# tanishqkumar/ssd

Measured on NVIDIA H100. Metric: decode tokens/sec (sync speculative decoding, accept-len reported), higher is better.
Workload: dtype bf16

## Files before the change

### ssd_b200/csrc/draft_stream.cuh

```cuda
#pragma once
#include "common.cuh"
#include "sampling.cuh"

namespace ssdk {

constexpr int kDsConsumers = 256;
constexpr int kDsWarps = kDsConsumers / 32;
constexpr int kDsThreads = kDsConsumers + 32;
constexpr int kDsMaxLayers = 32;
constexpr int kDsSplits = 16;
constexpr int kDsShortSplits = 8;
constexpr int kDsLongCtx = 256;
constexpr int kDsSlotBytes = 32768;
constexpr int kDsMaxSlots = 6;
constexpr int kDsMaxSteps = 8;
constexpr int kDsBtSmem = 32;

struct DsLayer {
  const __nv_bfloat16 *qkv, *o, *gate_up, *down, *in_norm, *post_norm, *q_norm, *k_norm;
};

struct DsParams {
  int d, L, H, KV, ffn, vocab, qk_norm;
  float eps, scale_log2;
// ... 11 lines not shown
  float* attn_part;
  __nv_bfloat16* logits;
  long long logits_ld;
  const float* temp;
  const uint64_t* dyn;
  uint64_t seed, call_base;
  ArgMax* samp_partial;
  unsigned* bar_state;
  unsigned* attn_ticket;
  int n_slots;
  DsLayer layers[kDsMaxLayers];
  const int64_t* pend_tok;
  __nv_bfloat16* vec_row0;
  const float* fp8_scale[kDsMaxLayers][4];
};

struct DsVecs {
  __nv_bfloat16 *qkv, *attn, *o, *down, *resid0, *resid1, *act;
  SSDK_DEVINL __nv_bfloat16* resid(int i) const { return i ? resid1 : resid0; }
};
SSDK_DEVINL DsVecs ds_row0_vecs(const DsParams& p, int hd) {
  DsVecs v{};
  __nv_bfloat16* b = p.vec_row0;
  if (!b) return v;
  v.qkv = b; b += ((p.H + 2 * p.KV) * hd + 7) / 8 * 8;
  v.attn = b; b += p.H * hd;
  v.o = b; b += p.d;
  v.down = b; b += p.d;
  v.resid0 = b; b += p.d;
  v.resid1 = b; b += p.d;
  v.act = b;
  return v;
}
__host__ SSDK_DEVINL int ds_xs_floats(int d, int ffn, int q_width) {
  const int a = 2 * d > ffn ? 2 * d : ffn;
  return a > q_width ? a : q_width;
}

SSDK_DEVINL void ds_sync() {
#ifdef SSDK_HOST_EMU
  ::emu::named_barrier(1, kDsConsumers);
#else
  asm volatile("bar.sync 1, 256;" ::: "memory");
#endif
}

struct DsGridBar {
  unsigned long long* counter;
  unsigned long long target;
  __device__ void init() {
    if (threadIdx.x == 0) {
      const unsigned long long c = ld_relaxed_gpu_u64(counter);
      target = c - c % (unsigned long long)gridDim.x;
    }
  }
  __device__ void sync() {
    ds_sync();
    if (threadIdx.x == 0) {
      target += (unsigned long long)gridDim.x;
      red_add_release_gpu_u64(counter, 1ull);
      const long long t0 = clock64();
      while (ld_relaxed_gpu_u64(counter) < target) {
        if (clock64() - t0 > 4000000000LL) __trap();
      }
      fence_acq_rel_gpu();
    }
    ds_sync();
  }
};
// ... 86 lines not shown
    const int parts = g.kind == DS_PAIR ? 2 : 1;
    for (int q = 0; q < parts; ++q) {
      const unsigned slot = n % S, round = n / S;
      mbar_wait(&empty[slot], (round & 1u) ^ 1u);
      mbar_arrive_expect_tx(&full[slot], bytes);
      const void* src = w + ((size_t)(q ? g.rows : 0) + (size_t)c.s * g.rpj) * g.K;
      if constexpr (FP8) {
        if (c.m != DS_HEAD)
          src = reinterpret_cast<const uint8_t*>(w) + ((size_t)(q ? g.rows : 0) + (size_t)c.s * g.rpj) * g.K;
      }
      bulk_load_g2s(ring + (size_t)slot * kDsSlotBytes, src, bytes, &full[slot]);
      ++n;
    }
    ds_cursor_next(p, geom, c);
  }
}

struct DsRing {
  uint8_t* base;
  uint64_t *full, *empty;
  unsigned n_slots;
  unsigned taken;
};
SSDK_DEVINL const uint8_t* ds_acquire(DsRing& r, unsigned k) {
  const unsigned n = r.taken + k, slot = n % r.n_slots;
  mbar_wait(&r.full[slot], (n / r.n_slots) & 1u);
  return r.base + (size_t)slot * kDsSlotBytes;
}
SSDK_DEVINL void ds_release(DsRing& r, unsigned k, int lane) {
  __syncwarp();
  if (lane == 0) mbar_arrive(&r.empty[(r.taken + k) % r.n_slots]);
}

SSDK_DEVINL void ds_load_x(const float* xseg, int steps, int lane, float (&xr)[kDsMaxSteps][8]) {
#pragma unroll
  for (int j = 0; j < kDsMaxSteps; ++j) {
    if (j < steps) {
      const float4 a = *reinterpret_cast<const float4*>(xseg + j * 256 + lane * 8);
      const float4 b = *reinterpret_cast<const float4*>(xseg + j * 256 + lane * 8 + 4);
      xr[j][0] = a.x; xr[j][1] = a.y; xr[j][2] = a.z; xr[j][3] = a.w;
      xr[j][4] = b.x; xr[j][5] = b.y; xr[j][6] = b.z; xr[j][7] = b.w;
    } else {
#pragma unroll
      for (int e = 0; e < 8; ++e) xr[j][e] = 0.f;
    }
  }
}
SSDK_DEVINL float ds_dot_seg(const uint8_t* wseg, int steps, int lane, const float (&xr)[kDsMaxSteps][8]) {
  const uint4* wp = reinterpret_cast<const uint4*>(wseg) + lane;
  float a0 = 0.f, a1 = 0.f, a2 = 0.f, a3 = 0.f;
#pragma unroll
  for (int j = 0; j < kDsMaxSteps; ++j) {
    if (j < steps) {
      const uint4 w = wp[j * 32];
      float2 f = ds_bf2(w.x);
      a0 = fmaf(f.x, xr[j][0], a0); a1 = fmaf(f.y, xr[j][1], a1);
      f = ds_bf2(w.y);
      a2 = fmaf(f.x, xr[j][2], a2); a3 = fmaf(f.y, xr[j][3], a3);
      f = ds_bf2(w.z);
      a0 = fmaf(f.x, xr[j][4], a0); a1 = fmaf(f.y, xr[j][5], a1);
      f = ds_bf2(w.w);
      a2 = fmaf(f.x, xr[j][6], a2); a3 = fmaf(f.y, xr[j][7], a3);
    }
  }
  return warp_sum((a0 + a1) + (a2 + a3));
}

SSDK_DEVINL float2 ds_e4m3x2(uint32_t v) {
#ifdef SSDK_HOST_EMU
  auto one = [](uint32_t b) {
    const int e = (int)((b >> 3) & 15u), m = (int)(b & 7u);
    float x = (e == 15 && m == 7) ? NAN : (e ? std::ldexp(1.0f + (float)m / 8.0f, e - 7) : std::ldexp((float)m, -9));
    return (b & 0x80u) ? -x : x;
  };
// ... 9 lines not shown
  const uint2* wp = reinterpret_cast<const uint2*>(wseg) + lane;
  float a0 = 0.f, a1 = 0.f, a2 = 0.f, a3 = 0.f;
#pragma unroll
  for (int j = 0; j < kDsMaxSteps; ++j) {
    if (j < steps) {
      const uint2 w = wp[j * 32];
      float2 f = ds_e4m3x2(w.x);
      a0 = fmaf(f.x, xr[j][0], a0); a1 = fmaf(f.y, xr[j][1], a1);
      f = ds_e4m3x2(w.x >> 16);
      a2 = fmaf(f.x, xr[j][2], a2); a3 = fmaf(f.y, xr[j][3], a3);
      f = ds_e4m3x2(w.y);
      a0 = fmaf(f.x, xr[j][4], a0); a1 = fmaf(f.y, xr[j][5], a1);
      f = ds_e4m3x2(w.y >> 16);
      a2 = fmaf(f.x, xr[j][6], a2); a3 = fmaf(f.y, xr[j][7], a3);
    }
  }
  return warp_sum((a0 + a1) + (a2 + a3));
}

struct DsSample {
  bool greedy;
  float invT;
  uint64_t seed, call_id;
  ArgMax best;
};
SSDK_DEVINL float ds_score(const DsSample& s, float logit, int idx) {
  if (s.greedy) return logit;
  const uint4 rnd = philox_draw((uint32_t)(idx >> 2), 0u, s.call_id, TAG_SAMPLE, s.seed);
  const float e = u32_to_exp1(u4_word(rnd, idx & 3)) + 1e-10f;
  return logit * s.invT - __logf(e);
}

struct DsRow0 {
  const float* xs;
  const __nv_bfloat16* xg;
  __nv_bfloat16* y;
};
SSDK_DEVINL float ds_dot_seg0(const uint8_t* wseg, int steps, int lane, const float* x0) {
  const uint4* wp = reinterpret_cast<const uint4*>(wseg) + lane;
  float a0 = 0.f, a1 = 0.f, a2 = 0.f, a3 = 0.f;
#pragma unroll 2
  for (int j = 0; j < steps; ++j) {
    const float4 u = *reinterpret_cast<const float4*>(x0 + j * 256 + lane * 8);
    const float4 v = *reinterpret_cast<const float4*>(x0 + j * 256 + lane * 8 + 4);
    const uint4 w = wp[j * 32];
    float2 f = ds_bf2(w.x);
    a0 = fmaf(f.x, u.x, a0); a1 = fmaf(f.y, u.y, a1);
    f = ds_bf2(w.y);
    a2 = fmaf(f.x, u.z, a2); a3 = fmaf(f.y, u.w, a3);
    f = ds_bf2(w.z);
    a0 = fmaf(f.x, v.x, a0); a1 = fmaf(f.y, v.y, a1);
    f = ds_bf2(w.w);
    a2 = fmaf(f.x, v.z, a2); a3 = fmaf(f.y, v.w, a3);
  }
  return warp_sum((a0 + a1) + (a2 + a3));
}
SSDK_DEVINL float ds_dot_seg08(const uint8_t* wseg, int steps, int lane, const float* x0) {
  const uint2* wp = reinterpret_cast<const uint2*>(wseg) + lane;
  float a0 = 0.f, a1 = 0.f, a2 = 0.f, a3 = 0.f;
#pragma unroll 2
  for (int j = 0; j < steps; ++j) {
    const float4 u = *reinterpret_cast<const float4*>(x0 + j * 256 + lane * 8);
    const float4 v = *reinterpret_cast<const float4*>(x0 + j * 256 + lane * 8 + 4);
    const uint2 w = wp[j * 32];
    float2 f = ds_e4m3x2(w.x);
    a0 = fmaf(f.x, u.x, a0); a1 = fmaf(f.y, u.y, a1);
    f = ds_e4m3x2(w.x >> 16);
    a2 = fmaf(f.x, u.z, a2); a3 = fmaf(f.y, u.w, a3);
    f = ds_e4m3x2(w.y);
    a0 = fmaf(f.x, v.x, a0); a1 = fmaf(f.y, v.y, a1);
    f = ds_e4m3x2(w.y >> 16);
    a2 = fmaf(f.x, v.z, a2); a3 = fmaf(f.y, v.w, a3);
  }
  return warp_sum((a0 + a1) + (a2 + a3));
}
SSDK_DEVINL void ds_load_vec(const __nv_bfloat16* v, int n, float* xs);
SSDK_DEVINL const float* ds_row0_x(const DsRow0& r, float* xs, int n) {
  if (r.xs) return r.xs;
  ds_sync();
  ds_load_vec(r.xg, n, xs);
  return xs;
}

template <bool HEAD, bool TWO = false>
SSDK_DEVINL void ds_consume_plain(DsRing& ring, const DsGeom& g, float* xs, __nv_bfloat16* y, DsSample* smp,
                                  const DsRow0& r0 = DsRow0{}) {
  static_assert(!(HEAD && TWO), "row 0 has no lm_head");
  if ((int)blockIdx.x >= g.nj) return;
  const int warp = threadIdx.x >> 5, lane = threadIdx.x & 31;
  const int steps = g.K >> 8;
  float xr[kDsMaxSteps][8];
  ds_load_x(xs, steps, lane, xr);
  const float* x0 = nullptr;
  if constexpr (TWO) x0 = ds_row0_x(r0, xs, g.K);
  for (int s = (int)blockIdx.x; s < g.nj; s += (int)gridDim.x) {
    const uint8_t* st = ds_acquire(ring, 0);
    const float acc = ds_dot_seg(st + (size_t)warp * g.K * 2, steps, lane, xr);
    float acc0 = 0.f;
    if constexpr (TWO) acc0 = ds_dot_seg0(st + (size_t)warp * g.K * 2, steps, lane, x0);
    ds_release(ring, 0, lane);
    ring.taken += 1u;
    const int row = s * 8 + warp;
    if (lane == 0 && row < g.rows) {
      const __nv_bfloat16 o = f2bf(acc);
      if (!HEAD) {
        y[row] = o;
        if constexpr (TWO) r0.y[row] = f2bf(acc0);
      } else {
        if (y) y[row] = o;
        smp->best = argmax_better(smp->best, ArgMax{ds_score(*smp, bf2f(o), row), row});
      }
    }
  }
}
SSDK_DEVINL float ds_silu_mul(float gate, float up) {
  gate = bf16_round(gate);
  up = bf16_round(up);
  return (gate / (1.0f + __expf(-gate))) * up;
}
template <bool TWO>
SSDK_DEVINL void ds_consume_pair(DsRing& ring, const DsGeom& g, float* xs, __nv_bfloat16* act, const DsRow0& r0) {
  if ((int)blockIdx.x >= g.nj) return;
  const int warp = threadIdx.x >> 5, lane = threadIdx.x & 31;
  const int steps = g.K >> 8;
  float xr[kDsMaxSteps][8];
  ds_load_x(xs, steps, lane, xr);
  const float* x0 = nullptr;
  if constexpr (TWO) x0 = ds_row0_x(r0, xs, g.K);
  for (int s = (int)blockIdx.x; s < g.nj; s += (int)gridDim.x) {
    float gate0 = 0.f, up0 = 0.f;
    const uint8_t* sg = ds_acquire(ring, 0);
    const float gate = ds_dot_seg(sg + (size_t)warp * g.K * 2, steps, lane, xr);
    if constexpr (TWO) gate0 = ds_dot_seg0(sg + (size_t)warp * g.K * 2, steps, lane, x0);
    ds_release(ring, 0, lane);
    const uint8_t* su = ds_acquire(ring, 1);
    const float up = ds_dot_seg(su + (size_t)warp * g.K * 2, steps, lane, xr);
    if constexpr (TWO) up0 = ds_dot_seg0(su + (size_t)warp * g.K * 2, steps, lane, x0);
    ds_release(ring, 1, lane);
    ring.taken += 2u;
    const int i = s * 8 + warp;
    if (lane == 0 && i < g.rows) {
      act[i] = f2bf(ds_silu_mul(gate, up));
      if constexpr (TWO) r0.y[i] = f2bf(ds_silu_mul(gate0, up0));
    }
  }
}
template <bool TWO>
SSDK_DEVINL void ds_consume_split(DsRing& ring, const DsGeom& g, float* xs, float* res, __nv_bfloat16* y,
                                  const DsRow0& r0) {
  if ((int)blockIdx.x >= g.nj) return;
  const int warp = threadIdx.x >> 5, lane = threadIdx.x & 31;
  const int row_in_job = warp / g.segs, seg = warp - row_in_job * g.segs;
  const int seg_len = g.K / g.segs, steps = seg_len >> 8;
  float xr[kDsMaxSteps][8];
  ds_load_x(xs + seg * seg_len, steps, lane, xr);
  const float* x0 = nullptr;
  if constexpr (TWO) x0 = ds_row0_x(r0, xs, g.K);
  const size_t w_off = ((size_t)row_in_job * g.K + (size_t)seg * seg_len) * 2;
  unsigned it = 0;
  for (int s = (int)blockIdx.x; s < g.nj; s += (int)gridDim.x, ++it) {
    const uint8_t* st = ds_acquire(ring, 0);
    const float acc = ds_dot_seg(st + w_off, steps, lane, xr);
    float acc0 = 0.f;
    if constexpr (TWO) acc0 = ds_dot_seg0(st + w_off, steps, lane, x0 + seg * seg_len);
    ds_release(ring, 0, lane);
    ring.taken += 1u;
    float* rb = res + (it & 1u) * kDsWarps;
    float* rb0 = rb + 2 * kDsWarps;
    if (lane == 0) {
      rb[warp] = acc;
      if constexpr (TWO) rb0[warp] = acc0;
    }
    ds_sync();
    if ((int)threadIdx.x < g.rpj) {
      const int row = s * g.rpj + (int)threadIdx.x;
      if (row < g.rows) {
        float v = 0.f;
        for (int q = 0; q < g.segs; ++q) v += rb[(int)threadIdx.x * g.segs + q];
        y[row] = f2bf(v);
        if constexpr (TWO) {
          float v0 = 0.f;
          for (int q = 0; q < g.segs; ++q) v0 += rb0[(int)threadIdx.x * g.segs + q];
          r0.y[row] = f2bf(v0);
        }
      }
    }
  }
}

template <bool TWO>
SSDK_DEVINL void ds_consume_plain8(DsRing& ring, const DsGeom& g, float* xs, __nv_bfloat16* y, const DsRow0& r0,
                                   const float* scale) {
  if ((int)blockIdx.x >= g.nj) return;
  const int warp = threadIdx.x >> 5, lane = threadIdx.x & 31;
  const int steps = g.K >> 8;
  float xr[kDsMaxSteps][8];
  ds_load_x(xs, steps, lane, xr);
  const float* x0 = nullptr;
  if constexpr (TWO) x0 = ds_row0_x(r0, xs, g.K);
  for (int s = (int)blockIdx.x; s < g.nj; s += (int)gridDim.x) {
    const int ra = s * 16 + warp, rb = ra + 8;
    const float sa = ra < g.rows ? scale[ra] : 0.f, sb = rb < g.rows ? scale[rb] : 0.f;
    const uint8_t* wa = ds_acquire(ring, 0) + (size_t)warp * g.K;
    const uint8_t* wb = wa + (size_t)8 * g.K;
    const float acc_a = ds_dot_seg8(wa, steps, lane, xr);
    const float acc_b = ds_dot_seg8(wb, steps, lane, xr);
    float acc0_a = 0.f, acc0_b = 0.f;
    if constexpr (TWO) {
      acc0_a = ds_dot_seg08(wa, steps, lane, x0);
      acc0_b = ds_dot_seg08(wb, steps, lane, x0);
    }
    ds_release(ring, 0, lane);
    ring.taken += 1u;
    if (lane == 0) {
      if (ra < g.rows) {
        y[ra] = f2bf(acc_a * sa);
        if constexpr (TWO) r0.y[ra] = f2bf(acc0_a * sa);
      }
      if (rb < g.rows) {
        y[rb] = f2bf(acc_b * sb);
        if constexpr (TWO) r0.y[rb] = f2bf(acc0_b * sb);
      }
    }
  }
}
template <bool TWO>
SSDK_DEVINL void ds_consume_pair8(DsRing& ring, const DsGeom& g, float* xs, __nv_bfloat16* act, const DsRow0& r0,
                                  const float* scale) {
  if ((int)blockIdx.x >= g.nj) return;
  const int warp = threadIdx.x >> 5, lane = threadIdx.x & 31;
  const int steps = g.K >> 8;
  float xr[kDsMaxSteps][8];
  ds_load_x(xs, steps, lane, xr);
  const float* x0 = nullptr;
  if constexpr (TWO) x0 = ds_row0_x(r0, xs, g.K);
  for (int s = (int)blockIdx.x; s < g.nj; s += (int)gridDim.x) {
    const int ia = s * 16 + warp, ib = ia + 8;
    const float sga = ia < g.rows ? scale[ia] : 0.f, sua = ia < g.rows ? scale[g.rows + ia] : 0.f;
    const float sgb = ib < g.rows ? scale[ib] : 0.f, sub = ib < g.rows ? scale[g.rows + ib] : 0.f;
    float ga0 = 0.f, gb0 = 0.f, ua0 = 0.f, ub0 = 0.f;
    const uint8_t* sg = ds_acquire(ring, 0) + (size_t)warp * g.K;
    const float ga = ds_dot_seg8(sg, steps, lane, xr);
    const float gb = ds_dot_seg8(sg + (size_t)8 * g.K, steps, lane, xr);
    if constexpr (TWO) {
      ga0 = ds_dot_seg08(sg, steps, lane, x0);
      gb0 = ds_dot_seg08(sg + (size_t)8 * g.K, steps, lane, x0);
    }
    ds_release(ring, 0, lane);
    const uint8_t* su = ds_acquire(ring, 1) + (size_t)warp * g.K;
    const float ua = ds_dot_seg8(su, steps, lane, xr);
    const float ub = ds_dot_seg8(su + (size_t)8 * g.K, steps, lane, xr);
    if constexpr (TWO) {
      ua0 = ds_dot_seg08(su, steps, lane, x0);
      ub0 = ds_dot_seg08(su + (size_t)8 * g.K, steps, lane, x0);
    }
    ds_release(ring, 1, lane);
    ring.taken += 2u;
    if (lane == 0) {
      if (ia < g.rows) {
        act[ia] = f2bf(ds_silu_mul(ga * sga, ua * sua));
        if constexpr (TWO) r0.y[ia] = f2bf(ds_silu_mul(ga0 * sga, ua0 * sua));
      }
      if (ib < g.rows) {
        act[ib] = f2bf(ds_silu_mul(gb * sgb, ub * sub));
        if constexpr (TWO) r0.y[ib] = f2bf(ds_silu_mul(gb0 * sgb, ub0 * sub));
      }
    }
  }
}
template <bool TWO>
SSDK_DEVINL void ds_consume_split8(DsRing& ring, const DsGeom& g, float* xs, float* res, __nv_bfloat16* y,
                                   const DsRow0& r0, const float* scale) {
  if ((int)blockIdx.x >= g.nj) return;
  const int warp = threadIdx.x >> 5, lane = threadIdx.x & 31;
  const int R = kDsWarps / g.segs;
  const int row_in_job = warp / g.segs, seg = warp - row_in_job * g.segs;
  const int seg_len = g.K / g.segs, steps = seg_len >> 8;
  float xr[kDsMaxSteps][8];
  ds_load_x(xs + seg * seg_len, steps, lane, xr);
  const float* x0 = nullptr;
  if constexpr (TWO) x0 = ds_row0_x(r0, xs, g.K) + seg * seg_len;
  const size_t off_a = (size_t)row_in_job * g.K + (size_t)seg * seg_len, off_b = off_a + (size_t)R * g.K;
  unsigned it = 0;
  for (int s = (int)blockIdx.x; s < g.nj; s += (int)gridDim.x, ++it) {
    const int row = s * g.rpj + (int)threadIdx.x;
    const float sc = ((int)threadIdx.x < g.rpj && row < g.rows) ? scale[row] : 0.f;
    const uint8_t* st = ds_acquire(ring, 0);
    const float acc_a = ds_dot_seg8(st + off_a, steps, lane, xr);
    const float acc_b = ds_dot_seg8(st + off_b, steps, lane, xr);
    float acc0_a = 0.f, acc0_b = 0.f;
    if constexpr (TWO) {
      acc0_a = ds_dot_seg08(st + off_a, steps, lane, x0);
      acc0_b = ds_dot_seg08(st + off_b, steps, lane, x0);
    }
    ds_release(ring, 0, lane);
    ring.taken += 1u;
    float* rb = res + (it & 1u) * 2 * kDsWarps;
    float* rb0 = rb + 4 * kDsWarps;
    if (lane == 0) {
      rb[warp] = acc_a;
      rb[kDsWarps + warp] = acc_b;
      if constexpr (TWO) {
        rb0[warp] = acc0_a;
        rb0[kDsWarps + warp] = acc0_b;
      }
    }
    ds_sync();
    if ((int)threadIdx.x < g.rpj && row < g.rows) {
      const int grp = (int)threadIdx.x / R;
      const int base = grp * kDsWarps + ((int)threadIdx.x - grp * R) * g.segs;
      float v = 0.f;
      for (int q = 0; q < g.segs; ++q) v += rb[base + q];
      y[row] = f2bf(v * sc);
      if constexpr (TWO) {
        float v0 = 0.f;
        for (int q = 0; q < g.segs; ++q) v0 += rb0[base + q];
        r0.y[row] = f2bf(v0 * sc);
      }
    }
  }
}

template <bool FP8 = false>
SSDK_DEVINL void ds_consume(DsRing& ring, const DsGeom& g, float* xs, float* res, __nv_bfloat16* y, bool two,
                            const DsRow0& r0, const float* scale = nullptr) {
  if constexpr (FP8) {
    if (g.kind == DS_PLAIN) {
      if (two) ds_consume_plain8<true>(ring, g, xs, y, r0, scale);
      else ds_consume_plain8<false>(ring, g, xs, y, r0, scale);
    } else {
      if (two) ds_consume_split8<true>(ring, g, xs, res, y, r0, scale);
      else ds_consume_split8<false>(ring, g, xs, res, y, r0, scale);
    }
  } else {
    if (g.kind == DS_PLAIN) {
      if (two) ds_consume_plain<false, true>(ring, g, xs, y, nullptr, r0);
      else ds_consume_plain<false>(ring, g, xs, y, nullptr);
    } else {
      if (two) ds_consume_split<true>(ring, g, xs, res, y, r0);
      else ds_consume_split<false>(ring, g, xs, res, y, r0);
    }
  }
}
template <bool FP8 = false>
SSDK_DEVINL void ds_consume_gu(DsRing& ring, const DsGeom& g, float* xs, __nv_bfloat16* act, bool two, const DsRow0& r0,
                               const float* scale = nullptr) {
  if constexpr (FP8) {
    if (two) ds_consume_pair8<true>(ring, g, xs, act, r0, scale);
    else ds_consume_pair8<false>(ring, g, xs, act, r0, scale);
  } else {
    if (two) ds_consume_pair<true>(ring, g, xs, act, r0);
    else ds_consume_pair<false>(ring, g, xs, act, r0);
  }
}

SSDK_DEVINL float ds_block_sum(float v, float* red) {
  const int lane = threadIdx.x & 31, wid = threadIdx.x >> 5;
  v = warp_sum(v);
  ds_sync();
  if (lane == 0) red[wid] = v;
  ds_sync();
  float t = (lane < kDsWarps) ? red[lane] : 0.f;
  return warp_sum(t);
}

struct DsPre {
  uint4 w, b;
};
SSDK_DEVINL DsPre ds_preload(const __nv_bfloat16* b, const __nv_bfloat16* w, int d) {
  DsPre r;
  const int i = threadIdx.x * 8;
  r.w = r.b = make_uint4(0u, 0u, 0u, 0u);
  if (i < d) {
    r.w = *reinterpret_cast<const uint4*>(w + i);
    if (b) r.b = ds_ldcg16(b + i);
  }
  return r;
}
SSDK_DEVINL void ds_norm_prologue(const __nv_bfloat16* a, const __nv_bfloat16* b, __nv_bfloat16* resid_out,
                                  const __nv_bfloat16* w, float eps, int d, float* xs, float* red, const DsPre* pre) {
  float ss = 0.f;
  const int i0 = threadIdx.x * 8;
  for (int i = i0; i < d; i += kDsConsumers * 8) {
    float x[8];
    unpack_bf16x8(ds_ldcg16(a + i), x);
    if (b) {
      float y[8];
      unpack_bf16x8((pre && i == i0) ? pre->b : ds_ldcg16(b + i), y);
#pragma unroll
      for (int j = 0; j < 8; ++j) x[j] += y[j];
    }
    if (resid_out && blockIdx.x == 0) *reinterpret_cast<uint4*>(resid_out + i) = pack_bf16x8(x);
#pragma unroll
    for (int j = 0; j < 8; ++j) {
      xs[i + j] = x[j];
      ss += x[j] * x[j];
    }
  }
  ss = ds_block_sum(ss, red);
  const float rstd = rsqrtf(ss / (float)d + eps);
  for (int i = i0; i < d; i += kDsConsumers * 8) {
    float wv[8];
    unpack_bf16x8((pre && i == i0) ? pre->w : *reinterpret_cast<const uint4*>(w + i), wv);
#pragma unroll
    for (int j = 0; j < 8; ++j) xs[i + j] = bf16_round(xs[i + j] * rstd * wv[j]);
  }
  ds_sync();
}
SSDK_DEVINL void ds_load_vec(const __nv_bfloat16* v, int n, float* xs) {
  for (int i = threadIdx.x * 8; i < n; i += kDsConsumers * 8) {
    float x[8];
    unpack_bf16x8(ds_ldcg16(v + i), x);
#pragma unroll
    for (int j = 0; j < 8; ++j) xs[i + j] = x[j];
  }
  ds_sync();
}

SSDK_DEVINL int ds_num_splits(int ctx) {
  return ctx > kDsLongCtx ? kDsSplits : min(kDsShortSplits, max(1, (ctx + 7) >> 3));
}
SSDK_DEVINL int ds_page_of(const DsParams& p, const int* bt_s, int t) {
  const int i = t / p.block_size;
  return p.max_blocks <= kDsBtSmem ? bt_s[i] : p.block_table[i];
}
template <int HD, int TB>
SSDK_DEVINL void ds_load_kv(const DsParams& p, const int* bt_s, const __nv_bfloat16* kbase, const __nv_bfloat16* vbase, int h,
                            int tb, int t1, int pos, int lane, float (&kv)[TB][HD / 32], float (&vv)[TB][HD / 32]) {
  constexpr int EPL = HD / 32;
  static_assert(EPL == 2 || EPL == 4, "head_dim 64 or 128");
#pragma unroll
  for (int u = 0; u < TB; ++u) {
    const int t = tb + u * kDsWarps;
#pragma unroll
    for (int e = 0; e < EPL; ++e) kv[u][e] = vv[u][e] = 0.f;
    if (t < t1 && t != pos) {
      const int blk = ds_page_of(p, bt_s, t);
      const size_t off = (((size_t)blk * p.block_size + t % p.block_size) * p.KV + h) * HD + lane * EPL;
      if constexpr (EPL == 2) {
        const float2 a = ds_bf2(__ldcg(reinterpret_cast<const uint32_t*>(kbase + off)));
        const float2 b = ds_bf2(__ldcg(reinterpret_cast<const uint32_t*>(vbase + off)));
        kv[u][0] = a.x; kv[u][1] = a.y; vv[u][0] = b.x; vv[u][1] = b.y;
      } else {
        const uint2 a = __ldcg(reinterpret_cast<const uint2*>(kbase + off));
        const uint2 b = __ldcg(reinterpret_cast<const uint2*>(vbase + off));
        float2 f = ds_bf2(a.x); kv[u][0] = f.x; kv[u][1] = f.y;
        f = ds_bf2(a.y); kv[u][EPL - 2] = f.x; kv[u][EPL - 1] = f.y;
        f = ds_bf2(b.x); vv[u][0] = f.x; vv[u][1] = f.y;
// ... 195 lines not shown
      }
      float o = 0.f, l = 0.f;
#pragma unroll
      for (int q = 0; q < kDsSplits; ++q) {
        const float wt = (ms[q] == -INFINITY) ? 0.f : exp2f(ms[q] - mx);
        o += os[q] * wt;
        l += ls[q] * wt;
      }
      vattn[(size_t)(h * G + g) * HD + dim] = f2bf(l > 0.f ? o / l : 0.f);
    }
  }
  ds_sync();
}


template <bool FP8>
SSDK_DEVINL const float* ds_scale(const DsParams& p, int l, int m) {
  if constexpr (FP8) return p.fp8_scale[l][m];
  else return nullptr;
}

template <int HD, int GMAX, bool FP8 = false>
__global__ void __launch_bounds__(kDsThreads, 1) draft_stream_kernel(const __grid_constant__ DsParams p) {
  SSDK_DYN_SMEM(uint8_t, ds_smem);
  SSDK_STATIC_SMEM(uint64_t, full_bar, kDsMaxSlots);
  SSDK_STATIC_SMEM(uint64_t, empty_bar, kDsMaxSlots);
  SSDK_STATIC_SMEM(DsGeom, geom, 5);
  SSDK_STATIC_SMEM(float, red, 32);
  SSDK_STATIC_SMEM(float, res, (FP8 ? 8 : 4) * kDsWarps);
  SSDK_STATIC_SMEM(ArgMax, ared, 32);
  SSDK_SHARED_VAR(int, tok_s);
  SSDK_SHARED_VAR(int, flag_s);
  SSDK_STATIC_SMEM(int, bt_s, kDsBtSmem);
  float* xs = reinterpret_cast<float*>(ds_smem + (size_t)p.n_slots * kDsSlotBytes);
  float* scratch = xs + ds_xs_floats(p.d, p.ffn, p.H * HD);
  if (threadIdx.x < kDsBtSmem && (int)threadIdx.x < p.max_blocks) bt_s[threadIdx.x] = p.block_table[threadIdx.x];
  if (threadIdx.x == 0) {
    trace_mark(TR_MISC);
    if constexpr (FP8) {
      ds_geometry8(p.d, (p.H + 2 * p.KV) * HD, false, &geom[DS_QKV]);
      ds_geometry8(p.H * HD, p.d, false, &geom[DS_O]);
      ds_geometry8(p.d, p.ffn, true, &geom[DS_GU]);
      ds_geometry8(p.ffn, p.d, false, &geom[DS_DOWN]);
    } else {
      ds_geometry(p.d, (p.H + 2 * p.KV) * HD, false, &geom[DS_QKV]);
      ds_geometry(p.H * HD, p.d, false, &geom[DS_O]);
      ds_geometry(p.d, p.ffn, true, &geom[DS_GU]);
      ds_geometry(p.ffn, p.d, false, &geom[DS_DOWN]);
    }
    ds_geometry(p.d, p.vocab, false, &geom[DS_HEAD]);
    for (int s = 0; s < p.n_slots; ++s) {
      mbar_init(&full_bar[s], 1);
      mbar_init(&empty_bar[s], kDsWarps);
    }
    fence_mbar_init();
  }
  __syncthreads();

  if (threadIdx.x >= kDsConsumers) {
    if (threadIdx.x == kDsConsumers) ds_producer<FP8>(p, geom, ds_smem, full_bar, empty_bar);
    return;
  }

  DsRing ring;
  ring.base = ds_smem;
  ring.full = full_bar;
  ring.empty = empty_bar;
  ring.n_slots = (unsigned)p.n_slots;
  ring.taken = 0u;
  DsGridBar bar;
  bar.counter = reinterpret_cast<unsigned long long*>(p.bar_state);
  bar.target = 0;
  bar.init();

  const int ctx_base = p.ctx0[0];
  const float T = p.temp ? p.temp[0] : 0.f;
  const uint64_t seed = p.dyn ? p.dyn[0] : p.seed;
  const uint64_t call0 = p.dyn ? p.dyn[1] * 16ull : p.call_base;
  __nv_bfloat16* resid[2] = {p.resid0, p.resid1};
  long long tok = p.tok_buf[0];
  const long long tok0 = p.pend_tok ? p.pend_tok[0] : -1;
  const DsVecs v0 = ds_row0_vecs(p, HD);

  for (int f = 0; f < p.n_fwd; ++f) {
    if (threadIdx.x == 0 && f > 0) trace_mark(TR_MISC);
    const int ctx = ctx_base + f + 1;
    const __nv_bfloat16* emb = p.embed + (size_t)tok * p.d;
    const bool two = f == 0 && tok0 >= 0;
    int cur = 0;
    DsPre pre;
    for (int l = 0; l < p.L; ++l) {
      const DsLayer& lw = p.layers[l];
      if (l == 0) {
        if (two) ds_norm_prologue(p.embed + (size_t)tok0 * p.d, nullptr, v0.resid(cur ^ 1), lw.in_norm, p.eps, p.d, xs + p.d, red,
                                  nullptr);
        ds_norm_prologue(emb, nullptr, resid[cur ^ 1], lw.in_norm, p.eps, p.d, xs, red, nullptr);
      } else {
        if (two) ds_norm_prologue(v0.down, v0.resid(cur), v0.resid(cur ^ 1), lw.in_norm, p.eps, p.d, xs + p.d, red, nullptr);
        ds_norm_prologue(p.vec_down, resid[cur], resid[cur ^ 1], lw.in_norm, p.eps, p.d, xs, red, &pre);
      }
      cur ^= 1;
      ds_mark(f, 0);
      ds_consume<FP8>(ring, geom[DS_QKV], xs, res, p.vec_qkv, two, DsRow0{xs + p.d, nullptr, v0.qkv},
                      ds_scale<FP8>(p, l, DS_QKV));
      ds_mark(f, 1);
      bar.sync();
      ds_mark(f, 2);
#ifdef SSDK_TRACE_FINE
      bar.sync();
      ds_mark(f, 12);
#endif
      if (two) {
        const int ns0 = ds_num_splits(ctx - 1);
        for (int u = blockIdx.x; u < p.KV * ns0; u += gridDim.x) {
          if (ns0 == kDsSplits)
            ds_attention_unit<HD, GMAX, 8>(p, v0.qkv, v0.attn, l, u / ns0, u % ns0, ns0, ctx - 1, scratch, &flag_s, bt_s);
          else ds_attention_unit<HD, GMAX, 4>(p, v0.qkv, v0.attn, l, u / ns0, u % ns0, ns0, ctx - 1, scratch, &flag_s, bt_s);
        }
        bar.sync();
      }
      const int ns = ds_num_splits(ctx);
      for (int u = blockIdx.x; u < p.KV * ns; u += gridDim.x) {
        if (ns == kDsSplits)
          ds_attention_unit<HD, GMAX, 8>(p, p.vec_qkv, p.vec_attn, l, u / ns, u % ns, ns, ctx, scratch, &flag_s, bt_s);
        else ds_attention_unit<HD, GMAX, 4>(p, p.vec_qkv, p.vec_attn, l, u / ns, u % ns, ns, ctx, scratch, &flag_s, bt_s);
      }
      ds_mark(f, 3);
      bar.sync();
      ds_mark(f, 4);
      ds_load_vec(p.vec_attn, p.H * HD, xs);
      ds_consume<FP8>(ring, geom[DS_O], xs, res, p.vec_o, two, DsRow0{nullptr, v0.attn, v0.o}, ds_scale<FP8>(p, l, DS_O));
      ds_mark(f, 5);
      pre = ds_preload(resid[cur], lw.post_norm, p.d);
      bar.sync();
      ds_mark(f, 6);
      if (two) ds_norm_prologue(v0.o, v0.resid(cur), v0.resid(cur ^ 1), lw.post_norm, p.eps, p.d, xs + p.d, red, nullptr);
      ds_norm_prologue(p.vec_o, resid[cur], resid[cur ^ 1], lw.post_norm, p.eps, p.d, xs, red, &pre);
      cur ^= 1;
      ds_mark(f, 7);
      ds_consume_gu<FP8>(ring, geom[DS_GU], xs, p.vec_act, two, DsRow0{xs + p.d, nullptr, v0.act},
                         ds_scale<FP8>(p, l, DS_GU));
      ds_mark(f, 8);
      bar.sync();
      ds_mark(f, 9);
      ds_load_vec(p.vec_act, p.ffn, xs);
      ds_consume<FP8>(ring, geom[DS_DOWN], xs, res, p.vec_down, two, DsRow0{nullptr, v0.act, v0.down},
                      ds_scale<FP8>(p, l, DS_DOWN));
      ds_mark(f, 10);
      pre = ds_preload(resid[cur], l + 1 < p.L ? p.layers[l + 1].in_norm : p.final_norm, p.d);
      bar.sync();
      ds_mark(f, 11);
    }
    if (!ds_has_head(p, f)) break;
    ds_norm_prologue(p.vec_down, resid[cur], nullptr, p.final_norm, p.eps, p.d, xs, red, &pre);
    DsSample smp;
    smp.greedy = (T == 0.f);
    smp.invT = smp.greedy ? 1.f : 1.f / T;
    smp.seed = seed;
    smp.call_id = call0 + (uint64_t)f;
    smp.best = ArgMax{-INFINITY, 0x7fffffff};
    ds_consume_plain<true>(ring, geom[DS_HEAD], xs, p.logits ? p.logits + (size_t)f * p.logits_ld : nullptr, &smp);
    if ((threadIdx.x & 31) == 0) ared[threadIdx.x >> 5] = smp.best;
    ds_sync();
    if (threadIdx.x == 0) {
      ArgMax b = ared[0];
      for (int w = 1; w < kDsWarps; ++w) b = argmax_better(b, ared[w]);
      p.samp_partial[blockIdx.x] = b;
    }
    bar.sync();
    {
      ArgMax a{-INFINITY, 0x7fffffff};
      for (int i = threadIdx.x; i < (int)gridDim.x; i += kDsConsumers) {
        ArgMax q;
        q.v = __ldcg(&p.samp_partial[i].v);
        q.i = __ldcg(&p.samp_partial[i].i);
        a = argmax_better(a, q);
      }
      a = warp_argmax(a);
      ds_sync();
      if ((threadIdx.x & 31) == 0) ared[threadIdx.x >> 5] = a;
      ds_sync();
      if (threadIdx.x == 0) {
        ArgMax b = ared[0];
        for (int w = 1; w < kDsWarps; ++w) b = argmax_better(b, ared[w]);
        tok_s = b.i;
      }
      ds_sync();
// ... 8 lines not shown
```

### ssd_b200/csrc/engine.cu

```cuda
#include <cuda.h>
#include <cuda_runtime.h>
#include <cudaTypedefs.h>
#include <nccl.h>

#include <algorithm>
#include <cstdarg>
#include <cstdio>
#include <cstdlib>
#include <cstring>
#include <map>
#include <string>
#include <tuple>
#include <vector>

#include "../../include/ssdk.h"
#include "attention.cuh"
#include "common.cuh"
#include "elementwise.cuh"
#include "gemm.cuh"
#include "sampling.cuh"
#include "draft_stream.cuh"

using namespace ssdk;
typedef __nv_bfloat16 bf16;
// ... 796 lines not shown
    tok_buf[(size_t)b * Kp1] = recovery[b];
    fold_ids[2 * b] = pend[b] >= 0 ? pend[b] : recovery[b];
    fold_ids[2 * b + 1] = recovery[b];
  }
}

__global__ void advance_kernel(int32_t* __restrict__ ctx, int64_t* __restrict__ recovery_in, int64_t* __restrict__ pend,
                               uint64_t* __restrict__ seed_step, const int64_t* __restrict__ tok_buf,
                               const int32_t* __restrict__ n_accept, const int64_t* __restrict__ recovery_out,
                               int64_t* __restrict__ log_tokens, int32_t* __restrict__ log_len, int B, int Kp1, int log_cap) {
  pdl_launch_dependents();
  pdl_wait();
  const int b = threadIdx.x;
  if (b < B) {
    const int n = n_accept[b] + 1;
    int len = log_len[b];
    for (int j = 0; j < n && len < log_cap; ++j) log_tokens[(size_t)b * log_cap + len++] = tok_buf[(size_t)b * Kp1 + j];
    log_len[b] = len;
    ctx[b] += n;
    recovery_in[b] = recovery_out[b];
    pend[b] = (n == Kp1) ? tok_buf[(size_t)b * Kp1 + Kp1 - 1] : -1;
  }
  if (threadIdx.x == 0) seed_step[1] += 1;
}

static bool draft_stream_enabled() {
  static int v = -1;
  if (v < 0) v = env_int("SSDK_DRAFT_STREAM", 1) != 0 ? 1 : 0;
  return v == 1;
}
constexpr int kMaxDynSmem = 227 * 1024 - 2048;
static size_t ds_fixed_smem(const Model& m) {
  const int G = m.H / m.KV, gmax = G <= 4 ? 4 : 8;
  const size_t xs = (size_t)ds_xs_floats(m.d, m.ffn, m.H * m.hd);
  const size_t scratch = (size_t)gmax * m.hd + 2 * m.hd + (size_t)kDsWarps * gmax * (m.hd + 2);
  return (xs + scratch) * 4 + 256;
}
static int ds_ring_slots(const Model& m) {
  const size_t fixed = ds_fixed_smem(m);
  if (fixed + 3 * (size_t)kDsSlotBytes > (size_t)kMaxDynSmem) return 0;
  return (int)std::min<size_t>(kDsMaxSlots, ((size_t)kMaxDynSmem - fixed) / kDsSlotBytes);
}
static bool draft_stream_supported(const Model& m, int B) {
  const int G = m.KV ? m.H / m.KV : 0;
  DsGeom g;
  return B == 1 && m.cfg.tp_size == 1 && m.cfg.layers <= kDsMaxLayers && (m.hd == 64 || m.hd == 128) && G >= 1 && G <= 8 &&
         m.H % m.KV == 0 && m.KV <= 32 && m.d % 8 == 0 && (m.H * m.hd) % 8 == 0 && m.ffn % 8 == 0 &&
         ds_geometry(m.d, m.qkv_dim, false, &g) && ds_geometry(m.H * m.hd, m.d, false, &g) &&
         ds_geometry(m.d, m.ffn, true, &g) && ds_geometry(m.ffn, m.d, false, &g) && ds_geometry(m.d, m.cfg.vocab, false, &g) &&
         ds_ring_slots(m) >= 3;
}
static int draft_stream_max_ctx() {
  static int v = -1;
  if (v < 0) v = std::max(0, env_int("SSDK_DRAFT_STREAM_MAX_CTX", 1024));
  return v;
}
static bool use_draft_stream(ssdk_engine* e, int B, int ctx_bound) {
  const Model& drf = e->model[SSDK_DRAFT];
  return drf.present && draft_stream_enabled() && draft_stream_supported(drf, B) &&
         ctx_bound + e->rt.spec_k + 1 <= draft_stream_max_ctx();
}
template <int HD, int GMAX, bool FP8>
static int launch_draft_stream(Launcher& L, const DsParams& p, size_t smem) {
  static bool attr_set = false;
  if (!attr_set) {
    CK(cudaFuncSetAttribute(draft_stream_kernel<HD, GMAX, FP8>, cudaFuncAttributeMaxDynamicSharedMemorySize, (int)smem));
    attr_set = true;
  }
  cudaLaunchConfig_t cfg = {};
  cfg.gridDim = dim3(num_sms());
  cfg.blockDim = dim3(kDsThreads);
  cfg.dynamicSmemBytes = smem;
  cfg.stream = L.st;
  cudaLaunchAttribute attr[1];
  attr[0].id = cudaLaunchAttributeCooperative;
  attr[0].val.cooperative = 1;
  cfg.attrs = attr;
  cfg.numAttrs = 1;
  cudaError_t err = cudaLaunchKernelEx(&cfg, draft_stream_kernel<HD, GMAX, FP8>, p);
  if (err != cudaSuccess) return fail("draft stream launch failed: %s", cudaGetErrorString(err));
  L.barrier_op();
  ++L.count;
  return 0;
}
static int enqueue_draft_stream(ssdk_engine* e, Launcher& L, int64_t* tok_buf, int n_fwd, const int64_t* pend,
                                const int32_t* ctx0, const int32_t* block_table, const float* temp, const uint64_t* dyn,
                                bf16* logits, int64_t logits_ld) {
  Model& m = e->model[SSDK_DRAFT];
  Workspace& w = e->ws;
  DsParams p;
  memset(&p, 0, sizeof(p));
  p.d = m.d; p.L = m.cfg.layers; p.H = m.H; p.KV = m.KV; p.ffn = m.ffn; p.vocab = m.cfg.vocab; p.qk_norm = m.cfg.qk_norm;
  p.eps = m.cfg.rms_eps;
  p.scale_log2 = (1.0f / sqrtf((float)m.hd)) * 1.4426950408889634f;
  p.embed = m.embed.ptr; p.final_norm = m.final_norm; p.lm_head = m.lm_head.ptr; p.rope = m.rope;
  p.k_cache = m.k_cache; p.v_cache = m.v_cache;
  p.cache_layer_stride = (long long)m.num_blocks * e->rt.block_size * m.KV * m.hd;
  p.block_size = e->rt.block_size; p.max_blocks = e->rt.max_blocks_per_seq;
  p.tok_buf = tok_buf; p.n_fwd = n_fwd; p.skip_last_head = 0;
  p.pend_tok = pend; p.vec_row0 = w.ds_vec0;
// ... 907 lines not shown
```

Before: 375.5.

## Store draft-stream activation vector in shared memory as bf16 instead of fp32

The normalized activation buffer xs in the persistent draft-stream kernel is now held in shared memory as bf16 rather than fp32, halving its footprint. Norm prologues stage fp32 values in the scratch region, and the consumers unpack bf16x8 with one 16-byte load instead of two float4 loads. The smaller fixed shared-memory size can leave room for more ring slots (up to the max of 6), which deepens weight prefetching. The kernel's smem attribute is now re-applied whenever a larger size is requested. Values were already rounded to bf16, so numerics should be unchanged.

Result: no change. 376.4, median of 6 (+0.3%).

```diff
diff --git a/ssd_b200/csrc/draft_stream.cuh b/ssd_b200/csrc/draft_stream.cuh
--- a/ssd_b200/csrc/draft_stream.cuh
+++ b/ssd_b200/csrc/draft_stream.cuh
@@ -67,9 +67,18 @@
   v.act = b;
   return v;
 }
-__host__ SSDK_DEVINL int ds_xs_floats(int d, int ffn, int q_width) {
+__host__ SSDK_DEVINL int ds_xs_elems(int d, int ffn, int q_width) {
   const int a = 2 * d > ffn ? 2 * d : ffn;
   return a > q_width ? a : q_width;
+}
+__host__ SSDK_DEVINL size_t ds_xs_bytes(int d, int ffn, int q_width) {
+  return ((size_t)ds_xs_elems(d, ffn, q_width) * 2 + 15) / 16 * 16;
+}
+__host__ SSDK_DEVINL int ds_xs_floats(int d, int ffn, int q_width) { return ds_xs_elems(d, ffn, q_width); }
+
+__host__ SSDK_DEVINL int ds_scratch_floats(int d, int hd, int gmax) {
+  const int att = gmax * hd + 2 * hd + kDsWarps * gmax * (hd + 2);
+  return att > d ? att : d;
 }
 
 SSDK_DEVINL void ds_sync() {
@@ -222,14 +231,11 @@
   if (lane == 0) mbar_arrive(&r.empty[(r.taken + k) % r.n_slots]);
 }
 
-SSDK_DEVINL void ds_load_x(const float* xseg, int steps, int lane, float (&xr)[kDsMaxSteps][8]) {
+SSDK_DEVINL void ds_load_x(const __nv_bfloat16* xseg, int steps, int lane, float (&xr)[kDsMaxSteps][8]) {
 #pragma unroll
   for (int j = 0; j < kDsMaxSteps; ++j) {
     if (j < steps) {
-      const float4 a = *reinterpret_cast<const float4*>(xseg + j * 256 + lane * 8);
-      const float4 b = *reinterpret_cast<const float4*>(xseg + j * 256 + lane * 8 + 4);
-      xr[j][0] = a.x; xr[j][1] = a.y; xr[j][2] = a.z; xr[j][3] = a.w;
-      xr[j][4] = b.x; xr[j][5] = b.y; xr[j][6] = b.z; xr[j][7] = b.w;
+      unpack_bf16x8(*reinterpret_cast<const uint4*>(xseg + j * 256 + lane * 8), xr[j]);
     } else {
 #pragma unroll
       for (int e = 0; e < 8; ++e) xr[j][e] = 0.f;
@@ -305,50 +311,48 @@
 }
 
 struct DsRow0 {
-  const float* xs;
+  const __nv_bfloat16* xs;
   const __nv_bfloat16* xg;
   __nv_bfloat16* y;
 };
-SSDK_DEVINL float ds_dot_seg0(const uint8_t* wseg, int steps, int lane, const float* x0) {
+SSDK_DEVINL float ds_dot_seg0(const uint8_t* wseg, int steps, int lane, const __nv_bfloat16* x0) {
   const uint4* wp = reinterpret_cast<const uint4*>(wseg) + lane;
   float a0 = 0.f, a1 = 0.f, a2 = 0.f, a3 = 0.f;
 #pragma unroll 2
   for (int j = 0; j < steps; ++j) {
-    const float4 u = *reinterpret_cast<const float4*>(x0 + j * 256 + lane * 8);
-    const float4 v = *reinterpret_cast<const float4*>(x0 + j * 256 + lane * 8 + 4);
+    const uint4 xv = *reinterpret_cast<const uint4*>(x0 + j * 256 + lane * 8);
     const uint4 w = wp[j * 32];
-    float2 f = ds_bf2(w.x);
+    float2 f = ds_bf2(w.x), u = ds_bf2(xv.x);
     a0 = fmaf(f.x, u.x, a0); a1 = fmaf(f.y, u.y, a1);
-    f = ds_bf2(w.y);
-    a2 = fmaf(f.x, u.z, a2); a3 = fmaf(f.y, u.w, a3);
-    f = ds_bf2(w.z);
-    a0 = fmaf(f.x, v.x, a0); a1 = fmaf(f.y, v.y, a1);
-    f = ds_bf2(w.w);
-    a2 = fmaf(f.x, v.z, a2); a3 = fmaf(f.y, v.w, a3);
+    f = ds_bf2(w.y); u = ds_bf2(xv.y);
+    a2 = fmaf(f.x, u.x, a2); a3 = fmaf(f.y, u.y, a3);
+    f = ds_bf2(w.z); u = ds_bf2(xv.z);
+    a0 = fmaf(f.x, u.x, a0); a1 = fmaf(f.y, u.y, a1);
+    f = ds_bf2(w.w); u = ds_bf2(xv.w);
+    a2 = fmaf(f.x, u.x, a2); a3 = fmaf(f.y, u.y, a3);
   }
   return warp_sum((a0 + a1) + (a2 + a3));
 }
-SSDK_DEVINL float ds_dot_seg08(const uint8_t* wseg, int steps, int lane, const float* x0) {
+SSDK_DEVINL float ds_dot_seg08(const uint8_t* wseg, int steps, int lane, const __nv_bfloat16* x0) {
   const uint2* wp = reinterpret_cast<const uint2*>(wseg) + lane;
   float a0 = 0.f, a1 = 0.f, a2 = 0.f, a3 = 0.f;
 #pragma unroll 2
   for (int j = 0; j < steps; ++j) {
-    const float4 u = *reinterpret_cast<const float4*>(x0 + j * 256 + lane * 8);
-    const float4 v = *reinterpret_cast<const float4*>(x0 + j * 256 + lane * 8 + 4);
+    const uint4 xv = *reinterpret_cast<const uint4*>(x0 + j * 256 + lane * 8);
     const uint2 w = wp[j * 32];
-    float2 f = ds_e4m3x2(w.x);
+    float2 f = ds_e4m3x2(w.x), u = ds_bf2(xv.x);
     a0 = fmaf(f.x, u.x, a0); a1 = fmaf(f.y, u.y, a1);
-    f = ds_e4m3x2(w.x >> 16);
-    a2 = fmaf(f.x, u.z, a2); a3 = fmaf(f.y, u.w, a3);
-    f = ds_e4m3x2(w.y);
-    a0 = fmaf(f.x, v.x, a0); a1 = fmaf(f.y, v.y, a1);
-    f = ds_e4m3x2(w.y >> 16);
-    a2 = fmaf(f.x, v.z, a2); a3 = fmaf(f.y, v.w, a3);
+    f = ds_e4m3x2(w.x >> 16); u = ds_bf2(xv.y);
+    a2 = fmaf(f.x, u.x, a2); a3 = fmaf(f.y, u.y, a3);
+    f = ds_e4m3x2(w.y); u = ds_bf2(xv.z);
+    a0 = fmaf(f.x, u.x, a0); a1 = fmaf(f.y, u.y, a1);
+    f = ds_e4m3x2(w.y >> 16); u = ds_bf2(xv.w);
+    a2 = fmaf(f.x, u.x, a2); a3 = fmaf(f.y, u.y, a3);
   }
   return warp_sum((a0 + a1) + (a2 + a3));
 }
-SSDK_DEVINL void ds_load_vec(const __nv_bfloat16* v, int n, float* xs);
-SSDK_DEVINL const float* ds_row0_x(const DsRow0& r, float* xs, int n) {
+SSDK_DEVINL void ds_load_vec(const __nv_bfloat16* v, int n, __nv_bfloat16* xs);
+SSDK_DEVINL const __nv_bfloat16* ds_row0_x(const DsRow0& r, __nv_bfloat16* xs, int n) {
   if (r.xs) return r.xs;
   ds_sync();
   ds_load_vec(r.xg, n, xs);
@@ -356,7 +360,7 @@
 }
 
 template <bool HEAD, bool TWO = false>
-SSDK_DEVINL void ds_consume_plain(DsRing& ring, const DsGeom& g, float* xs, __nv_bfloat16* y, DsSample* smp,
+SSDK_DEVINL void ds_consume_plain(DsRing& ring, const DsGeom& g, __nv_bfloat16* xs, __nv_bfloat16* y, DsSample* smp,
                                   const DsRow0& r0 = DsRow0{}) {
   static_assert(!(HEAD && TWO), "row 0 has no lm_head");
   if ((int)blockIdx.x >= g.nj) return;
@@ -364,7 +368,7 @@
   const int steps = g.K >> 8;
   float xr[kDsMaxSteps][8];
   ds_load_x(xs, steps, lane, xr);
-  const float* x0 = nullptr;
+  const __nv_bfloat16* x0 = nullptr;
   if constexpr (TWO) x0 = ds_row0_x(r0, xs, g.K);
   for (int s = (int)blockIdx.x; s < g.nj; s += (int)gridDim.x) {
     const uint8_t* st = ds_acquire(ring, 0);
@@ -392,13 +396,14 @@
   return (gate / (1.0f + __expf(-gate))) * up;
 }
 template <bool TWO>
-SSDK_DEVINL void ds_consume_pair(DsRing& ring, const DsGeom& g, float* xs, __nv_bfloat16* act, const DsRow0& r0) {
+SSDK_DEVINL void ds_consume_pair(DsRing& ring, const DsGeom& g, __nv_bfloat16* xs, __nv_bfloat16* act,
+                                 const DsRow0& r0) {
   if ((int)blockIdx.x >= g.nj) return;
   const int warp = threadIdx.x >> 5, lane = threadIdx.x & 31;
   const int steps = g.K >> 8;
   float xr[kDsMaxSteps][8];
   ds_load_x(xs, steps, lane, xr);
-  const float* x0 = nullptr;
+  const __nv_bfloat16* x0 = nullptr;
   if constexpr (TWO) x0 = ds_row0_x(r0, xs, g.K);
   for (int s = (int)blockIdx.x; s < g.nj; s += (int)gridDim.x) {
     float gate0 = 0.f, up0 = 0.f;
@@ -419,7 +424,7 @@
   }
 }
 template <bool TWO>
-SSDK_DEVINL void ds_consume_split(DsRing& ring, const DsGeom& g, float* xs, float* res, __nv_bfloat16* y,
+SSDK_DEVINL void ds_consume_split(DsRing& ring, const DsGeom& g, __nv_bfloat16* xs, float* res, __nv_bfloat16* y,
                                   const DsRow0& r0) {
   if ((int)blockIdx.x >= g.nj) return;
   const int warp = threadIdx.x >> 5, lane = threadIdx.x & 31;
@@ -427,7 +432,7 @@
   const int seg_len = g.K / g.segs, steps = seg_len >> 8;
   float xr[kDsMaxSteps][8];
   ds_load_x(xs + seg * seg_len, steps, lane, xr);
-  const float* x0 = nullptr;
+  const __nv_bfloat16* x0 = nullptr;
   if constexpr (TWO) x0 = ds_row0_x(r0, xs, g.K);
   const size_t w_off = ((size_t)row_in_job * g.K + (size_t)seg * seg_len) * 2;
   unsigned it = 0;
@@ -462,14 +467,14 @@
 }
 
 template <bool TWO>
-SSDK_DEVINL void ds_consume_plain8(DsRing& ring, const DsGeom& g, float* xs, __nv_bfloat16* y, const DsRow0& r0,
+SSDK_DEVINL void ds_consume_plain8(DsRing& ring, const DsGeom& g, __nv_bfloat16* xs, __nv_bfloat16* y, const DsRow0& r0,
                                    const float* scale) {
   if ((int)blockIdx.x >= g.nj) return;
   const int warp = threadIdx.x >> 5, lane = threadIdx.x & 31;
   const int steps = g.K >> 8;
   float xr[kDsMaxSteps][8];
   ds_load_x(xs, steps, lane, xr);
-  const float* x0 = nullptr;
+  const __nv_bfloat16* x0 = nullptr;
   if constexpr (TWO) x0 = ds_row0_x(r0, xs, g.K);
   for (int s = (int)blockIdx.x; s < g.nj; s += (int)gridDim.x) {
     const int ra = s * 16 + warp, rb = ra + 8;
@@ -498,14 +503,14 @@
   }
 }
 template <bool TWO>
-SSDK_DEVINL void ds_consume_pair8(DsRing& ring, const DsGeom& g, float* xs, __nv_bfloat16* act, const DsRow0& r0,
-                                  const float* scale) {
+SSDK_DEVINL void ds_consume_pair8(DsRing& ring, const DsGeom& g, __nv_bfloat16* xs, __nv_bfloat16* act,
+                                  const DsRow0& r0, const float* scale) {
   if ((int)blockIdx.x >= g.nj) return;
   const int warp = threadIdx.x >> 5, lane = threadIdx.x & 31;
   const int steps = g.K >> 8;
   float xr[kDsMaxSteps][8];
   ds_load_x(xs, steps, lane, xr);
-  const float* x0 = nullptr;
+  const __nv_bfloat16* x0 = nullptr;
   if constexpr (TWO) x0 = ds_row0_x(r0, xs, g.K);
   for (int s = (int)blockIdx.x; s < g.nj; s += (int)gridDim.x) {
     const int ia = s * 16 + warp, ib = ia + 8;
@@ -542,7 +547,7 @@
   }
 }
 template <bool TWO>
-SSDK_DEVINL void ds_consume_split8(DsRing& ring, const DsGeom& g, float* xs, float* res, __nv_bfloat16* y,
+SSDK_DEVINL void ds_consume_split8(DsRing& ring, const DsGeom& g, __nv_bfloat16* xs, float* res, __nv_bfloat16* y,
                                    const DsRow0& r0, const float* scale) {
   if ((int)blockIdx.x >= g.nj) return;
   const int warp = threadIdx.x >> 5, lane = threadIdx.x & 31;
@@ -551,7 +556,7 @@
   const int seg_len = g.K / g.segs, steps = seg_len >> 8;
   float xr[kDsMaxSteps][8];
   ds_load_x(xs + seg * seg_len, steps, lane, xr);
-  const float* x0 = nullptr;
+  const __nv_bfloat16* x0 = nullptr;
   if constexpr (TWO) x0 = ds_row0_x(r0, xs, g.K) + seg * seg_len;
   const size_t off_a = (size_t)row_in_job * g.K + (size_t)seg * seg_len, off_b = off_a + (size_t)R * g.K;
   unsigned it = 0;
@@ -595,7 +600,7 @@
 }
 
 template <bool FP8 = false>
-SSDK_DEVINL void ds_consume(DsRing& ring, const DsGeom& g, float* xs, float* res, __nv_bfloat16* y, bool two,
+SSDK_DEVINL void ds_consume(DsRing& ring, const DsGeom& g, __nv_bfloat16* xs, float* res, __nv_bfloat16* y, bool two,
                             const DsRow0& r0, const float* scale = nullptr) {
   if constexpr (FP8) {
     if (g.kind == DS_PLAIN) {
@@ -616,8 +621,8 @@
   }
 }
 template <bool FP8 = false>
-SSDK_DEVINL void ds_consume_gu(DsRing& ring, const DsGeom& g, float* xs, __nv_bfloat16* act, bool two, const DsRow0& r0,
-                               const float* scale = nullptr) {
+SSDK_DEVINL void ds_consume_gu(DsRing& ring, const DsGeom& g, __nv_bfloat16* xs, __nv_bfloat16* act, bool two,
+                               const DsRow0& r0, const float* scale = nullptr) {
   if constexpr (FP8) {
     if (two) ds_consume_pair8<true>(ring, g, xs, act, r0, scale);
     else ds_consume_pair8<false>(ring, g, xs, act, r0, scale);
@@ -651,7 +656,8 @@
   return r;
 }
 SSDK_DEVINL void ds_norm_prologue(const __nv_bfloat16* a, const __nv_bfloat16* b, __nv_bfloat16* resid_out,
-                                  const __nv_bfloat16* w, float eps, int d, float* xs, float* red, const DsPre* pre) {
+                                  const __nv_bfloat16* w, float eps, int d, __nv_bfloat16* xs, float* rs, float* red,
+                                  const DsPre* pre) {
   float ss = 0.f;
   const int i0 = threadIdx.x * 8;
   for (int i = i0; i < d; i += kDsConsumers * 8) {
@@ -666,7 +672,7 @@
     if (resid_out && blockIdx.x == 0) *reinterpret_cast<uint4*>(resid_out + i) = pack_bf16x8(x);
 #pragma unroll
     for (int j = 0; j < 8; ++j) {
-      xs[i + j] = x[j];
+      rs[i + j] = x[j];
       ss += x[j] * x[j];
     }
   }
@@ -676,17 +682,13 @@
     float wv[8];
     unpack_bf16x8((pre && i == i0) ? pre->w : *reinterpret_cast<const uint4*>(w + i), wv);
 #pragma unroll
-    for (int j = 0; j < 8; ++j) xs[i + j] = bf16_round(xs[i + j] * rstd * wv[j]);
+    for (int j = 0; j < 8; ++j) wv[j] = bf16_round(rs[i + j] * rstd * wv[j]);
+    *reinterpret_cast<uint4*>(xs + i) = pack_bf16x8(wv);
   }
   ds_sync();
 }
-SSDK_DEVINL void ds_load_vec(const __nv_bfloat16* v, int n, float* xs) {
-  for (int i = threadIdx.x * 8; i < n; i += kDsConsumers * 8) {
-    float x[8];
-    unpack_bf16x8(ds_ldcg16(v + i), x);
-#pragma unroll
-    for (int j = 0; j < 8; ++j) xs[i + j] = x[j];
-  }
+SSDK_DEVINL void ds_load_vec(const __nv_bfloat16* v, int n, __nv_bfloat16* xs) {
+  for (int i = threadIdx.x * 8; i < n; i += kDsConsumers * 8) *reinterpret_cast<uint4*>(xs + i) = ds_ldcg16(v + i);
   ds_sync();
 }
 
@@ -948,8 +950,8 @@
   SSDK_SHARED_VAR(int, tok_s);
   SSDK_SHARED_VAR(int, flag_s);
   SSDK_STATIC_SMEM(int, bt_s, kDsBtSmem);
-  float* xs = reinterpret_cast<float*>(ds_smem + (size_t)p.n_slots * kDsSlotBytes);
-  float* scratch = xs + ds_xs_floats(p.d, p.ffn, p.H * HD);
+  __nv_bfloat16* xs = reinterpret_cast<__nv_bfloat16*>(ds_smem + (size_t)p.n_slots * kDsSlotBytes);
+  float* scratch = reinterpret_cast<float*>(ds_smem + (size_t)p.n_slots * kDsSlotBytes + ds_xs_bytes(p.d, p.ffn, p.H * HD));
   if (threadIdx.x < kDsBtSmem && (int)threadIdx.x < p.max_blocks) bt_s[threadIdx.x] = p.block_table[threadIdx.x];
   if (threadIdx.x == 0) {
     trace_mark(TR_MISC);
@@ -1008,12 +1010,13 @@
     for (int l = 0; l < p.L; ++l) {
       const DsLayer& lw = p.layers[l];
       if (l == 0) {
-        if (two) ds_norm_prologue(p.embed + (size_t)tok0 * p.d, nullptr, v0.resid(cur ^ 1), lw.in_norm, p.eps, p.d, xs + p.d, red,
-                                  nullptr);
-        ds_norm_prologue(emb, nullptr, resid[cur ^ 1], lw.in_norm, p.eps, p.d, xs, red, nullptr);
+        if (two) ds_norm_prologue(p.embed + (size_t)tok0 * p.d, nullptr, v0.resid(cur ^ 1), lw.in_norm, p.eps, p.d, xs + p.d,
+                                  scratch, red, nullptr);
+        ds_norm_prologue(emb, nullptr, resid[cur ^ 1], lw.in_norm, p.eps, p.d, xs, scratch, red, nullptr);
       } else {
-        if (two) ds_norm_prologue(v0.down, v0.resid(cur), v0.resid(cur ^ 1), lw.in_norm, p.eps, p.d, xs + p.d, red, nullptr);
-        ds_norm_prologue(p.vec_down, resid[cur], resid[cur ^ 1], lw.in_norm, p.eps, p.d, xs, red, &pre);
+        if (two)
+          ds_norm_prologue(v0.down, v0.resid(cur), v0.resid(cur ^ 1), lw.in_norm, p.eps, p.d, xs + p.d, scratch, red, nullptr);
+        ds_norm_prologue(p.vec_down, resid[cur], resid[cur ^ 1], lw.in_norm, p.eps, p.d, xs, scratch, red, &pre);
       }
       cur ^= 1;
       ds_mark(f, 0);
@@ -1050,8 +1053,9 @@
       pre = ds_preload(resid[cur], lw.post_norm, p.d);
       bar.sync();
       ds_mark(f, 6);
-      if (two) ds_norm_prologue(v0.o, v0.resid(cur), v0.resid(cur ^ 1), lw.post_norm, p.eps, p.d, xs + p.d, red, nullptr);
-      ds_norm_prologue(p.vec_o, resid[cur], resid[cur ^ 1], lw.post_norm, p.eps, p.d, xs, red, &pre);
+      if (two)
+        ds_norm_prologue(v0.o, v0.resid(cur), v0.resid(cur ^ 1), lw.post_norm, p.eps, p.d, xs + p.d, scratch, red, nullptr);
+      ds_norm_prologue(p.vec_o, resid[cur], resid[cur ^ 1], lw.post_norm, p.eps, p.d, xs, scratch, red, &pre);
       cur ^= 1;
       ds_mark(f, 7);
       ds_consume_gu<FP8>(ring, geom[DS_GU], xs, p.vec_act, two, DsRow0{xs + p.d, nullptr, v0.act},
@@ -1068,7 +1072,7 @@
       ds_mark(f, 11);
     }
     if (!ds_has_head(p, f)) break;
-    ds_norm_prologue(p.vec_down, resid[cur], nullptr, p.final_norm, p.eps, p.d, xs, red, &pre);
+    ds_norm_prologue(p.vec_down, resid[cur], nullptr, p.final_norm, p.eps, p.d, xs, scratch, red, &pre);
     DsSample smp;
     smp.greedy = (T == 0.f);
     smp.invT = smp.greedy ? 1.f : 1.f / T;
diff --git a/ssd_b200/csrc/engine.cu b/ssd_b200/csrc/engine.cu
--- a/ssd_b200/csrc/engine.cu
+++ b/ssd_b200/csrc/engine.cu
@@ -852,9 +852,7 @@
 constexpr int kMaxDynSmem = 227 * 1024 - 2048;
 static size_t ds_fixed_smem(const Model& m) {
   const int G = m.H / m.KV, gmax = G <= 4 ? 4 : 8;
-  const size_t xs = (size_t)ds_xs_floats(m.d, m.ffn, m.H * m.hd);
-  const size_t scratch = (size_t)gmax * m.hd + 2 * m.hd + (size_t)kDsWarps * gmax * (m.hd + 2);
-  return (xs + scratch) * 4 + 256;
+  return ds_xs_bytes(m.d, m.ffn, m.H * m.hd) + (size_t)ds_scratch_floats(m.d, m.hd, gmax) * 4 + 256;
 }
 static int ds_ring_slots(const Model& m) {
   const size_t fixed = ds_fixed_smem(m);
@@ -882,10 +880,10 @@
 }
 template <int HD, int GMAX, bool FP8>
 static int launch_draft_stream(Launcher& L, const DsParams& p, size_t smem) {
-  static bool attr_set = false;
-  if (!attr_set) {
+  static size_t attr_smem = 0;
+  if (smem > attr_smem) {
     CK(cudaFuncSetAttribute(draft_stream_kernel<HD, GMAX, FP8>, cudaFuncAttributeMaxDynamicSharedMemorySize, (int)smem));
-    attr_set = true;
+    attr_smem = smem;
   }
   cudaLaunchConfig_t cfg = {};
   cfg.gridDim = dim3(num_sms());
```
